# jayleicn/ClipBERT

Measured on AMD Instinct MI355X. Metric: clips/sec/node (2×2 frames, 224px, L_txt=32) at 1/2/4/8 MI355X, higher is better.
Workload: dtype bf16; 1 GPU; MSRVTT retrieval training step (msrvtt_ret_base_resnet50.json; BASELINE configs[1]/[2] family) at the metric's shape: 16 videos x N_clip=2 x N_frame=2 uint8 frames 224px + 2 texts/video (pos+neg, r=2) L_txt=32 per GPU = 32 clips, 64 frames, 64 (text, clip) pairs per step; ImageNorm + fwd + lse-pooling loss + bwd + all-reduce + clip + AdamW in the timed step; clips folded into one forward; mode=train, videos_per_gpu=16, n_clips=2, n_frames=2, img_size=224, txt_len=32, texts_per_video=2, pairs_per_gpu=64, score_agg_func=lse, clips_folded=True, input=uint8 frames in HBM, parallelism=dp1, hip_graph=True, replay_plan=eager hyper-parameter upload + one hipGraph, n_graphs=1, dropout=True

## Files before the change

clipbert_amd/csrc/common.hip:

```cpp
#include "common.h"

#include <stdarg.h>
#include <stdio.h>

namespace {
thread_local char g_err[512] = "";
}

int cb_fail(const char* fmt, ...) {
    va_list ap;
    va_start(ap, fmt);
    vsnprintf(g_err, sizeof(g_err), fmt, ap);
    va_end(ap);
    return -1;
}

int cb_launch_status(const char* what) {
    hipError_t e = hipGetLastError();
    if (e != hipSuccess) return cb_fail("%s: kernel launch failed: %s", what, hipGetErrorString(e));
    return 0;
}

extern "C" const char* cb_last_error(void) { return g_err; }
extern "C" int cb_version(void) { return 18; }
```

clipbert_amd/csrc/gemm.hip:

```cpp

#include "gemm8_impl.h"
#include "gemm_stream_impl.h"
#include <stdio.h>
#include <vector>

using namespace cbgemm;

namespace cbgemm {
extern template int launch_gemm<float, 64, 64, 2>(const GP&, bool, hipStream_t);
extern template int launch_gemm<bf16, 128, 128, 2>(const GP&, bool, hipStream_t);
extern template int launch_gemm<bf16, 128, 64, 2>(const GP&, bool, hipStream_t);
extern template int launch_gemm<bf16, 64, 64, 3>(const GP&, bool, hipStream_t);
extern template int launch_gemm<bf16, 128, 128, 1, 2>(const GP&, bool, hipStream_t);
extern template int launch_gemm_group<float, 64, 64, 2, 1>(const GroupArgs&, int, hipStream_t);
extern template int launch_gemm_group<bf16, 64, 64, 3, 1>(const GroupArgs&, int, hipStream_t);
extern template int launch_gemm_group<bf16, 128, 128, 1, 2>(const GroupArgs&, int, hipStream_t);
#define CB_G8_DECL(BM, BN, WGM, WGN, NST)                                                             \
    extern template int launch_gemm8_fwd<BM, BN, WGM, WGN, NST>(const GP&, int, float*, hipStream_t);   \
    extern template int launch_gemm8_dgrad<BM, BN, WGM, WGN, NST>(const GP&, int, float*, hipStream_t); \
    extern template int launch_gemm8_wgrad<BM, BN, WGM, WGN, NST>(const GP&, int, float*, hipStream_t);
CB_G8_DECL(256, 256, 2, 4, 2)
CB_G8_DECL(128, 256, 2, 4, 3)
CB_G8_DECL(256, 128, 4, 2, 3)
#undef CB_G8_DECL
// ... 208 lines not shown
    const int taps = p.R * p.S;
    const bool tapped = d->a_mode == CB_ROWK_GATHER || d->b_mode == CB_KROW_TAPS || d->b_mode == CB_KROW_GATHER;
    if (tapped) {
        CB_REQUIRE(p.Ct > 0, "cb_gemm: Cin (channels per tap) must be set for conv modes");
        CB_REQUIRE(p.Ct % eps == 0, "cb_gemm: channels per tap (%d) must be a multiple of %d", p.Ct, eps);
    }
    const int64_t lim = 0x7fffffffll;
    bool fast = d->a_bytes > 0 && d->b_bytes > 0 && d->a_bytes < lim && d->b_bytes < lim && aligned16(d->A) && aligned16(d->B);
    if (d->a_mode == CB_ROWK_GATHER) {
        CB_REQUIRE(d->a_tab, "cb_gemm: a_tab missing");
        CB_REQUIRE(d->K == taps * p.Ct, "cb_gemm: K (%d) != R*S*Cin (%d)", d->K, taps * p.Ct);
        fast = fast && (p.R == 1 || d->sH % eps == 0) && (p.S == 1 || d->sW % eps == 0);
    } else if (d->a_mode == CB_ROWK) {
        fast = fast && (d->lda % eps == 0) && (d->K % eps == 0);
    } else {
        const int64_t need = ((int64_t)(d->K - 1) * d->lda + (d->M + eps - 1) / eps * eps) * esz;
        fast = fast && (d->lda % eps == 0) && (d->M % eps == 0 || need <= d->a_bytes);
    }
    if (d->b_mode == CB_ROWK) {
        fast = fast && (d->ldb % eps == 0) && (d->K % eps == 0);
    } else if (d->b_mode == CB_KROW) {
        const int64_t need = ((int64_t)(d->K - 1) * d->ldb + (d->N + eps - 1) / eps * eps) * esz;
        fast = fast && (d->ldb % eps == 0) && (d->N % eps == 0 || need <= d->b_bytes);
    } else if (d->b_mode == CB_KROW_TAPS) {
        CB_REQUIRE(d->K == taps * p.Ct, "cb_gemm: K (%d) != R*S*Ct (%d)", d->K, taps * p.Ct);
        fast = fast && (d->ldb % eps == 0) && (d->N % eps == 0);
    } else {
        CB_REQUIRE(d->b_tab, "cb_gemm: b_tab missing");
        CB_REQUIRE(d->N == taps * p.Ct, "cb_gemm: N (%d) != R*S*Cin (%d)", d->N, taps * p.Ct);
        fast = fast && (p.R == 1 || d->sH % eps == 0) && (p.S == 1 || d->sW % eps == 0);
    }
    p.a_bytes = (uint32_t)(fast ? d->a_bytes : 0);
    p.b_bytes = (uint32_t)(fast ? d->b_bytes : 0);
    CB_REQUIRE(d->tile >= 0 && d->tile <= 9, "cb_gemm: bad tile %d", d->tile);
    CB_REQUIRE(d->xcd_order >= 0 && d->xcd_order <= 2, "cb_gemm: bad xcd_order %d", d->xcd_order);
    CB_REQUIRE(d->dropout_p >= 0.f && d->dropout_p < 1.f, "cb_gemm: dropout_p out of range");
    const int cesz = d->c_f32 ? 4 : esz;
    bool cv = (d->ldc % 4 == 0) && ((reinterpret_cast<uintptr_t>(d->C) % (4 * cesz)) == 0);
    if (d->C2) cv = cv && (d->ldc2 % 4 == 0) && ((reinterpret_cast<uintptr_t>(d->C2) % (4 * esz)) == 0);
    if (d->residual) cv = cv && (d->ldr % 4 == 0) && ((reinterpret_cast<uintptr_t>(d->residual) % (4 * esz)) == 0);
    if (d->mask) cv = cv && (d->ldm % 4 == 0) && ((reinterpret_cast<uintptr_t>(d->mask) % (4 * esz)) == 0);
    if (d->gelu_grad_pre) cv = cv && (d->ld_gelu % 4 == 0) && ((reinterpret_cast<uintptr_t>(d->gelu_grad_pre) % (4 * esz)) == 0);
    if (d->scale) cv = cv && aligned16(d->scale);
    if (d->shift) cv = cv && aligned16(d->shift);
    p.c_vec = cv;
    bool cv8 = cv && (d->N % 8 == 0) && (d->ldc % 8 == 0) && aligned16(d->C);
    if (d->C2) cv8 = cv8 && (d->ldc2 % 8 == 0) && aligned16(d->C2);
    if (d->residual) cv8 = cv8 && (d->ldr % 8 == 0) && aligned16(d->residual);
    if (d->mask) cv8 = cv8 && (d->ldm % 8 == 0) && aligned16(d->mask);
    if (d->gelu_grad_pre) cv8 = cv8 && (d->ld_gelu % 8 == 0) && aligned16(d->gelu_grad_pre);
    out.fast = fast; out.cv8 = cv8;
    out.form = operand_form(d->a_mode, d->b_mode, taps); out.taps = taps;
    out.epi_scale_only = !d->C2 && !d->residual && !d->mask && !d->gelu_grad_pre && d->act == CB_ACT_NONE && !d->relu_after && !d->shift && d->dropout_p <= 0.f;
    out.atomics_ok = out.epi_scale_only && d->c_f32 && d->accumulate == 1;
    return 0;
}

int gemm_validate(const cb_gemm_desc* d, Prepared& pr, bool& empty) {
    empty = false;
    CB_REQUIRE(d != nullptr, "cb_gemm: null descriptor");
    CB_REQUIRE(d->M >= 0 && d->N >= 0 && d->K >= 0, "cb_gemm: negative dims");
    empty = d->M == 0 || d->N == 0;
    return empty ? 0 : gemm_prepare(d, pr);
}

void trace_plan(const cb_gemm_desc* d, const Prepared& pr, const LaunchPlan& lp) {
    if (lp.tile == 9)
        fprintf(stderr, "cb_gemm: M=%d N=%d K=%d modes=%d/%d tile=9 (asked %d) few rows\n", d->M, d->N, d->K, d->a_mode, d->b_mode, d->tile);
    else if (lp.tile == 8)
        fprintf(stderr, "cb_gemm: M=%d N=%d K=%d modes=%d/%d tile=8 (asked %d) stream variant %d\n", d->M, d->N, d->K, d->a_mode, d->b_mode, d->tile, lp.sched);
    else
        fprintf(stderr, "cb_gemm: M=%d N=%d K=%d modes=%d/%d tile=%d (asked %d) form8=%d split=%d ws=%d\n", d->M, d->N, d->K, d->a_mode, d->b_mode,
                lp.picked, d->tile, lp.form8, lp.tile >= 5 ? lp.split_k : pr.p.split_k, (int)lp.slab);
}

int gemm_launch(const cb_gemm_desc* d, const Prepared& pr, const LaunchPlan& lp, hipStream_t st) {
    GP p = pr.p;
    if (lp.tile == 9) return launch_gemm_skinny(d, p, st);
    p.split_k = lp.split_k;
    p.c_vec8 = lp.c_vec8;
    p.xcd_remap = lp.xcd_remap;
    if (lp.tile == 8) return launch_gemm_stream(p, lp.sched, st);
    if (lp.tile >= 5) {
        float* ws = lp.slab ? reinterpret_cast<float*>(d->splitk_ws) : nullptr;
        CB_STAMP_ASSIGN(p, d, lp.tile, p.split_k, lp.sched, 0, 1);
        int rc;
        if (lp.tile == 5) rc = launch8<256, 256, 2, 4, 2>(lp.form8, p, lp.sched - 1, ws, st);
        else if (lp.tile == 6) rc = launch8<128, 256, 2, 4, 3>(lp.form8, p, lp.sched - 1, ws, st);
        else rc = launch8<256, 128, 4, 2, 3>(lp.form8, p, lp.sched - 1, ws, st);
        if (rc != 0 || !ws) return rc;
        GP q = p;
        q.split_k = 1;
        const int64_t chunks = (int64_t)d->M * (d->N / 8);
        hipLaunchKernelGGL(splitk_reduce_kernel, dim3((unsigned)((chunks + 255) / 256), (unsigned)p.batch), dim3(256), 0, st, q, ws, p.split_k);
        return cb_launch_status("cb_gemm (split-K reduce)");
    }
    if (d->dtype == CB_F32) return launch_gemm<float, 64, 64, 2>(p, pr.fast, st);
    CB_STAMP_ASSIGN(p, d, lp.tile, p.split_k, 0, 0, 1);
    if (lp.tile == 4) return launch_gemm<bf16, 128, 128, 1, 2>(p, pr.fast, st);
    if (lp.tile == 1) return launch_gemm<bf16, 128, 128, 2>(p, pr.fast, st);
    if (lp.tile == 3) return launch_gemm<bf16, 128, 64, 2>(p, pr.fast, st);
    return launch_gemm<bf16, 64, 64, 3>(p, pr.fast, st);
}

int gemm_run(const cb_gemm_desc* d, const Prepared& pr, void* stream) {
    LaunchPlan lp;
    const int rc = gemm_choose(d, pr, true, false, lp);
    if (lp.tile != 0 && switches().trace) trace_plan(d, pr, lp);
    return rc != 0 ? rc : gemm_launch(d, pr, lp, cb_stream(stream));
}
}

extern "C" int cb_gemm(const cb_gemm_desc* d, void* stream) {
    Prepared pr;
    bool empty;
// ... 241 lines not shown
```

clipbert_amd/csrc/gemm_choose.h:

```cpp
#pragma once
#include "gemm_impl.h"
#include <cmath>
#include "gemm_tuned.h"
#include "gemm_model.h"

namespace cbgemm {
bool skinny_covers(const cb_gemm_desc* d, const GP& p);
}
using namespace cbgemm;

namespace {
inline int env_int(const char* name, int dflt) { const char* v = getenv(name); return v != nullptr ? atoi(v) : dflt; }
struct Switches {
    bool trace = getenv("CB_GEMM_TRACE") != nullptr;
    bool no_tuned = getenv("CB_GEMM_NO_TUNED") != nullptr;
    bool no_model = getenv("CB_GEMM_NO_MODEL") != nullptr;
    bool no_xcd_remap = getenv("CB_GEMM_NO_XCD_REMAP") != nullptr;
    bool no_stream = getenv("CB_GEMM_NO_STREAM") != nullptr;
    bool no_group = getenv("CB_GEMM_NO_GROUP") != nullptr;
    bool no_skinny = getenv("CB_GEMM_NO_SKINNY") != nullptr;
    bool group_slab_off = env_int("CB_GROUP_SLAB", 1) == 0;
    bool fast_epi_off = env_int("CB_GEMM_FAST_EPI", 1) == 0;
    int wt = env_int("CB_GEMM_WT", 1);
};
// ... 71 lines not shown
    for (int ti = 0; ti < 4; ++ti) {
        if (N <= 64 && ti >= 2) continue;
        consider(ti, split_caller, 0);
        if (free_split)
            for (int s : SPLITS4)
                if (s != split_caller && s <= (p.ktiles / 4 > 1 ? p.ktiles / 4 : 1)) consider(ti, s, 0);
    }
    if (can8)
        for (int ti = 4; ti < 7; ++ti) {
            const int64_t tiles = ((M + MODEL_BM[ti] - 1) / MODEL_BM[ti]) * ((N + MODEL_BN[ti] - 1) / MODEL_BN[ti]) * batch;
            int cand[3] = {1, 0, 0};
            int n = 1;
            for (int target : {256, 512}) {
                const int s = (int)std::lround((double)target / (double)tiles);
                if (s > 1 && p.ktiles / s >= 2 && (int64_t)s * batch * M * N * 4 <= ws_bytes && s != cand[1]) cand[n++] = s;
            }
            for (int i = 0; i < n; ++i) { consider(ti, cand[i], 1); consider(ti, cand[i], 3); }
        }
    return best;
}

int stream_variant(const cb_gemm_desc* d, const Prepared& pr) {
    const GP& p = pr.p;
    if (!pr.fast || !pr.cv8 || d->dtype != CB_BF16 || pr.form != FORM_FWD || p.batch > 1 || p.split_k > 1) return -1;
    if (d->c_f32 || d->accumulate || d->c_rowmap || d->zero_fill_pitch || d->a_rowsum || d->gelu_grad_pre || d->dropout_p > 0.f || d->mask || d->relu_bwd ||
        d->C2 || d->res_rowmap) return -1;
    if (d->K % 8 != 0 || d->M < 64) return -1;
    if ((int64_t)d->M * (d->N > d->K ? d->N : d->K) * 2 >= 0x7fffffffll) return -1;
    if (p.ktiles == 1 && d->N % 256 == 0) return 0;
    if (p.ktiles == 2 && d->N % 128 == 0) return 1;
    return -1;
}

struct LaunchPlan {
    int tile = 0;
    int split_k = 1;
    int sched = 0;
    bool xcd_remap = false;
    bool slab = false;
    bool c_vec8 = false;
    int form8 = 0;
    int picked = 0;
};
struct Pick { int tile = 0, split = 0, sched = 0; };
constexpr int64_t WS_UNLIMITED = (int64_t)1 << 60;
constexpr int STREAM_MIN_ROWS = 32768;

int gemm_choose(const cb_gemm_desc* d, const Prepared& pr, bool use_table, bool assume_ws, LaunchPlan& lp) {
    const Switches& sw = switches();
    const GP& p = pr.p;
    const bool bf = d->dtype == CB_BF16, explicit_tile = d->tile != 0;
    const int split_caller = p.split_k;
    lp = LaunchPlan{};
    const bool covers9 = skinny_covers(d, p);
    CB_REQUIRE(d->tile != 9 || covers9, "cb_gemm: tile 9 (few rows) does not cover this problem (bf16, A k-contiguous, B k-contiguous or aligned reduction-major, no batch / K split / row sums)");
    if (d->tile == 9 || (!explicit_tile && use_table && !sw.no_skinny && covers9 && d->M <= 64)) { lp.tile = 9; return 0; }
    const int sv = stream_variant(d, pr);
    CB_REQUIRE(d->tile != 8 || sv >= 0, "cb_gemm: tile 8 (streaming) does not cover this problem (M=%d N=%d K=%d modes %d/%d)", d->M, d->N, d->K, d->a_mode, d->b_mode);
    const cbgemm::TunedEntry* tabled =
        (bf && use_table && !sw.no_tuned && !d->dgrad_s2) ? cbgemm::tuned_lookup(d->a_mode, d->b_mode, d->M, d->N, d->K, p.batch, pr.taps, split_caller) : nullptr;
    if (!tabled && bf && use_table && !sw.no_tuned && pr.form == FORM_FWD)
        tabled = cbgemm::tuned_lookup(CB_ROWK_GATHER, d->b_mode, d->M, d->N, d->K, p.batch, 1, split_caller);
    if (d->tile == 8 || (!explicit_tile && use_table && !sw.no_stream && !tabled && sv >= 0 && d->M >= STREAM_MIN_ROWS && d->N <= 512)) {
        lp.tile = 8; lp.sched = sv; lp.c_vec8 = true;
        return 0;
    }

    const int form8 = (bf && pr.fast && pr.cv8 && (pr.form != FORM_DGRAD_TAPS || p.Ct % 64 == 0) && !d->res_rowmap && !d->dgrad_s2) ? FORM8_OF[pr.form] : 0;
    const int64_t ws_room = assume_ws ? splitk_payload_bytes(WS_UNLIMITED)
                                      : (d->splitk_ws && aligned16(d->splitk_ws) ? splitk_payload_bytes(d->splitk_ws_bytes) : 0);
    const bool free_split = !explicit_tile && a_reduction_major(pr.form) && pr.atomics_ok;
    const int xcd = d->xcd_order != 0 ? d->xcd_order : (tabled ? tabled->xcd : 0);
    auto model = [&](bool allow8) {
        Pick k;
        if (!bf || sw.no_model) return k;
        const ModelPick mp = model_pick(d, pr, allow8 && form8 != 0, ws_room, free_split && !d->a_rowsum && p.batch == 1);
        k.tile = mp.tile; k.split = (mp.tile >= 5 || mp.split != split_caller) ? mp.split : 0; k.sched = mp.sched;
        return k;
    };
    auto split8 = [&](const Pick& k) { return explicit_tile ? split_caller : (k.split > 0 ? k.split : 1); };
    Pick pick;
    if (explicit_tile) pick.tile = d->tile;
    else if (tabled) pick = Pick{tabled->tile, tabled->new_split, tabled->sched};
    if (pick.tile >= 5 && form8 == 0) pick = Pick{};
    if (pick.tile == 0) pick = model(true);
    if (pick.tile >= 5 && d->sq_slots && split8(pick) > 1) pick = model(false);
    if (pick.tile >= 5) {
        int split = split8(pick);
        if (split > p.ktiles) split = p.ktiles;
// ... 42 lines not shown
```

clipbert_amd/csrc/gemm_impl.h:

```cpp
#pragma once
#include "common.h"
#include <stdlib.h>
#include <type_traits>

namespace cbgemm {


constexpr int NTHREADS = 256;

template <typename T> struct Tr;
template <> struct Tr<bf16> { static constexpr int EPS = 8, BK = 64, SEGS = 8, ROWB = 128, RB = 8; };
template <> struct Tr<float> { static constexpr int EPS = 4, BK = 32, SEGS = 8, ROWB = 144, RB = 4; };

template <typename T> __device__ __forceinline__ int lds_off(int row, int seg);
template <> __device__ __forceinline__ int lds_off<bf16>(int row, int seg) { return row * 128 + ((seg ^ (row & 7)) << 4); }
template <> __device__ __forceinline__ int lds_off<float>(int row, int seg) { return row * 144 + (seg << 4); }

struct GP {
    const void* A; const void* B; void* C; void* C2; const void* residual; const void* mask;
    const void* dact_pre; float* a_rowsum; int64_t ldd;
    int relu_bwd;
    int cls_rows;
    const float* post_scale; const float* post_scale2;
    int batch;
// ... 640 lines not shown

__device__ __forceinline__ void apply_batch(GP& p, TileId& t) {
    if (p.batch <= 1) return;
    const int b = __builtin_amdgcn_readfirstlane(t.bz / p.split_k);
    t.bz -= b * p.split_k;
    const int64_t oa = b * p.bs_a, ob = b * p.bs_b;
    p.A = reinterpret_cast<const unsigned char*>(p.A) + oa;
    p.B = reinterpret_cast<const unsigned char*>(p.B) + ob;
    p.C = reinterpret_cast<unsigned char*>(p.C) + b * p.bs_c;
    if (p.a_bytes) p.a_bytes -= (uint32_t)oa;
    if (p.b_bytes) p.b_bytes -= (uint32_t)ob;
    if (p.a_rowsum) p.a_rowsum += b * p.bs_r;
}

template <int BM, int BK>
__device__ __forceinline__ void dgrad_s2_class(GP& p, TileId& bid) {
    if (p.cls_rows <= 0) return;
    const int cls = 3 - (bid.by & 3);
    bid.by >>= 2;
    const int py = cls >> 1, px = cls & 1;
    p.M = p.cls_rows;
    p.R = 1 + py; p.S = 1 + px;
    p.K = p.R * p.S * p.Ct;
    p.ktiles = (p.K + BK - 1) / BK;
    p.flip = TAP_S2 + 3 * (1 + py) + (1 + px);
    p.c_rowmap += (int64_t)cls * p.cls_rows;
}
inline int dgrad_s2_grid_y(const GP& p, int BM) { return p.cls_rows > 0 ? 4 * ((p.cls_rows + BM - 1) / BM) : (p.M + BM - 1) / BM; }

}
#include "gemm_epilogue.h"
namespace cbgemm {

template <typename T, int BM, int BN, typename LA, typename LB, int PF, bool RS, int OCC>
__device__ __forceinline__ void gemm_tile(GP& p, TileId bid, float* slab = nullptr, int* cnt = nullptr) {
    using X = Tr<T>;
    constexpr int BK = X::BK;
    constexpr int WM = BM / 2, WN = BN / 2, FM = WM / 16, FN = WN / 16;
    constexpr int TILE_A = BM * X::ROWB, TILE_B = BN * X::ROWB;
    constexpr int SMEM_BYTES = 2 * (TILE_A + TILE_B);
    __shared__ __attribute__((aligned(16))) unsigned char smem[SMEM_BYTES];

    const int tid = threadIdx.x, lane = tid & 63, wave = tid >> 6;
    const int wm = wave >> 1, wn = wave & 1;
    CB_STAMP_DECL();
    CB_STAMP(0);
#ifdef CB_STAMPS
    const unsigned stamp_lin = (unsigned)bid.bx + (unsigned)((p.N + BN - 1) / BN) * ((unsigned)bid.by + (unsigned)((p.M + BM - 1) / BM) * (unsigned)bid.bz);
#endif
    const int tile_lin = ((p.batch > 1 ? bid.bz / p.split_k : 0) * ((p.M + BM - 1) / BM) + bid.by) * ((p.N + BN - 1) / BN) + bid.bx;
    apply_batch(p, bid);
    if constexpr (!LA::KROW && LB::KROW) dgrad_s2_class<BM, BK>(p, bid);
    const int m0 = bid.by * BM, n0 = bid.bx * BN;
    const int kt_per = (p.ktiles + p.split_k - 1) / p.split_k;
    const int kt0 = bid.bz * kt_per;
    const int nt = ((kt0 + kt_per < p.ktiles) ? kt0 + kt_per : p.ktiles) - kt0;
    if (nt <= 0) return;

    LA la;
    LB lb;
    {
        Opnd oa = {p.A, p.a_tab, p.lda, p.a_mode, p.a_bytes};
        Opnd ob = {p.B, p.b_tab, p.ldb, p.b_mode, p.b_bytes};
        la.init(p, oa, m0, p.M, kt0, tid);
        lb.init(p, ob, n0, p.N, kt0, tid);
    }
    typename LA::Stage sa[PF];
    typename LB::Stage sb[PF];

    auto load_tiles = [&](typename LA::Stage& xa, typename LB::Stage& xb) {
        la.template load<false>(xa, p);
        lb.template load<false>(xb, p);
    };
    auto load_tiles_checked = [&](typename LA::Stage& xa, typename LB::Stage& xb) {
        la.template load<true>(xa, p);
        lb.template load<true>(xb, p);
    };
    auto store_tiles = [&](const typename LA::Stage& xa, const typename LB::Stage& xb, int buf) {
        unsigned char* As = smem + buf * (TILE_A + TILE_B);
        la.store(xa, As, tid);
        lb.store(xb, As + TILE_A, tid);
    };

    f32x4 acc[FM][FN];
#pragma unroll
    for (int i = 0; i < FM; ++i)
#pragma unroll
        for (int j = 0; j < FN; ++j) { f32x4 z = {0.f, 0.f, 0.f, 0.f}; acc[i][j] = z; }
    f32x4 accr[RS ? FM : 1];
#pragma unroll
    for (int i = 0; i < (RS ? FM : 1); ++i) { f32x4 z = {0.f, 0.f, 0.f, 0.f}; accr[i] = z; }
    const bool rs_on = RS && p.a_rowsum != nullptr && bid.bx == 0 && wn == 0;

#pragma unroll
    for (int s = 0; s < PF; ++s)
        if (s < nt) load_tiles_checked(sa[s], sb[s]);
    constexpr bool DGRAD = sizeof(T) == 2 && !LA::KROW && LB::KROW;
    constexpr int EPF = !DGRAD ? 0 : (BM * BN <= 128 * 64 ? 2 : (OCC >= 2 ? 1 : 0));
    EpiPre<BM, BN, EPF != 1> epre;
    const bool epf_on = EPF != 0 && p.c_vec8 && (EPF == 2 ? p.relu_bwd != 0 : (p.dact_pre != nullptr && !p.relu_bwd));
    if constexpr (EPF != 0) {
        if (epf_on) epi_prefetch<T, BM, BN, EPF != 1>(p, epre, m0, n0, tid);
    }
    store_tiles(sa[0], sb[0], 0);
    if (PF < nt) load_tiles_checked(sa[0], sb[0]);
    __syncthreads();
    CB_STAMP(1);

    auto compute_tile = [&](int buf) {
        const unsigned char* As = smem + buf * (TILE_A + TILE_B);
        const unsigned char* Bs = As + TILE_A;
        if constexpr (sizeof(T) == 2) {
#pragma unroll
            for (int kk = 0; kk < BK / 32; ++kk) {
                bf16x8 af[FM], bfr[FN];
#pragma unroll
                for (int i = 0; i < FM; ++i) {
                    if constexpr (LA::TR) af[i] = tr_frag<BM>(As, wm * WM + i * 16, kk, lane);
                    else af[i] = *reinterpret_cast<const bf16x8*>(As + lds_off<T>(wm * WM + i * 16 + (lane & 15), kk * 4 + (lane >> 4)));
                }
#pragma unroll
                for (int j = 0; j < FN; ++j) {
                    if constexpr (LB::TR) bfr[j] = tr_frag<BN>(Bs, wn * WN + j * 16, kk, lane);
                    else bfr[j] = *reinterpret_cast<const bf16x8*>(Bs + lds_off<T>(wn * WN + j * 16 + (lane & 15), kk * 4 + (lane >> 4)));
                }
#pragma unroll
                for (int i = 0; i < FM; ++i)
#pragma unroll
                    for (int j = 0; j < FN; ++j)
                        acc[i][j] = __builtin_amdgcn_mfma_f32_16x16x32_bf16(bfr[j], af[i], acc[i][j], 0, 0, 0);
                if constexpr (RS) {
// ... 39 lines not shown
            compute_tile(t & 1);
            store_tiles(sa[S1], sb[S1], (t + 1) & 1);
            load_tiles(sa[S1], sb[S1]);
            __syncthreads();
            ++t;
        }
    }
    while (t < nt) {
#pragma unroll
        for (int s = 0; s < PF; ++s) {
            if (t < nt) {
                const int S1 = (s + 1) % PF;
                compute_tile(t & 1);
                if (t + 1 < nt) {
                    store_tiles(sa[S1], sb[S1], (t + 1) & 1);
                    if (t + 1 + PF < nt) load_tiles_checked(sa[S1], sb[S1]);
                }
                __syncthreads();
                ++t;
            }
        }
    }

    if constexpr (RS) {
        if (rs_on && (lane >> 4) == 0) {
#pragma unroll
            for (int i = 0; i < FM; ++i) {
                const int m = m0 + wm * WM + i * 16 + lane;
                if (m < p.M) atomicAdd(p.a_rowsum + m, accr[i][0]);
            }
        }
    }
    CB_STAMP(2);
    if (slab != nullptr && p.split_k > 1) {
        __shared__ int s_last;
        constexpr int SC1 = 16;
        const int tile_lin = bid.by * ((p.N + BN - 1) / BN) + bid.bx;
        const int parts = (p.ktiles + kt_per - 1) / kt_per;
        float* const base = slab + ((int64_t)p.slab_base + (int64_t)tile_lin * p.split_k) * (BM * BN);
        {
            const rsrc_t rs = __builtin_amdgcn_make_buffer_rsrc(base + (int64_t)bid.bz * (BM * BN), (short)0, BM * BN * 4, 0x00020000);
#pragma unroll
            for (int i = 0; i < BM / 32; ++i)
#pragma unroll
                for (int j = 0; j < BN / 32; ++j) {
                    union { f32x4 f; u32x4 r; } u;
                    u.f = acc[i][j];
                    __builtin_amdgcn_raw_buffer_store_b128(u.r, rs, (uint32_t)(((i * (BN / 32) + j) * NTHREADS + tid) * 16), 0, SC1);
                }
        }
        __builtin_amdgcn_s_waitcnt(0x0f70);
        __syncthreads();
        if (tid == 0) s_last = atomicAdd(cnt + p.cnt_base + tile_lin, 1) == parts - 1;
        __syncthreads();
        if (!s_last) {
            CB_STAMP(3);
            CB_STAMP_FLUSH(p, stamp_lin, tid);
            return;
        }
#pragma unroll
        for (int i = 0; i < BM / 32; ++i)
#pragma unroll
            for (int j = 0; j < BN / 32; ++j) { f32x4 z = {0.f, 0.f, 0.f, 0.f}; acc[i][j] = z; }
#pragma unroll 2
        for (int z = 0; z < parts; ++z) {
            const rsrc_t rs = __builtin_amdgcn_make_buffer_rsrc(base + (int64_t)z * (BM * BN), (short)0, BM * BN * 4, 0x00020000);
#pragma unroll
            for (int i = 0; i < BM / 32; ++i)
#pragma unroll
                for (int j = 0; j < BN / 32; ++j) {
                    union { u32x4 r; f32x4 f; } u;
                    u.r = __builtin_amdgcn_raw_buffer_load_b128(rs, (uint32_t)(((i * (BN / 32) + j) * NTHREADS + tid) * 16), 0, SC1);
                    acc[i][j] += u.f;
                }
        }
        if (tid == 0) atomicExch(cnt + p.cnt_base + tile_lin, 0);
        p.split_k = 1;
    }
    constexpr int FORM_ = LA::KROW ? 0 : (LB::KROW ? 2 : 1);
    if constexpr (EPF != 0) tile_epilogue<T, BM, BN, SMEM_BYTES, EPF, false, FORM_>(p, acc, smem, m0, n0, tid, epre, epf_on);
    else tile_epilogue<T, BM, BN, SMEM_BYTES, 0, LA::KROW, FORM_>(p, acc, smem, m0, n0, tid, EpiPre<BM, BN, true>{}, false, tile_lin);
    CB_STAMP(3);
    CB_STAMP_FLUSH(p, stamp_lin, tid);
}

template <typename T, int BM, int BN, typename LA, typename LB, int PF, bool RS = false, int OCC = 1>
__global__ void __launch_bounds__(256, OCC) gemm_kernel(GP p) {
    gemm_tile<T, BM, BN, LA, LB, PF, RS, OCC>(p, tile_id(p));
}

#ifdef CB_STAMPS
constexpr int GROUP_MAX = 9;
#else
constexpr int GROUP_MAX = 10;
#endif
struct GroupArgs {
    int n, xcd_remap;
    int tile_end[GROUP_MAX];
    float* slab;
    int* cnt;
    GP g[GROUP_MAX];
};
static_assert(sizeof(GroupArgs) + 256 <= 4096, "kernel arguments (+ the hidden ones) are limited to 4 KiB");

template <int BM, int BN>
__device__ __forceinline__ int group_locate(const GroupArgs& ga, TileId& bid) {
    const unsigned total = gridDim.x;
    unsigned lin = blockIdx.x;
    if (ga.xcd_remap) {
        const unsigned xcd = lin & 7u, i = lin >> 3;
        const unsigned q = total >> 3, r = total & 7u;
        lin = (xcd < r ? xcd * (q + 1) : r * (q + 1) + (xcd - r) * q) + i;
    }
    int pi = 0;
    while (pi + 1 < ga.n && lin >= (unsigned)ga.tile_end[pi]) ++pi;
    const unsigned local = lin - (pi > 0 ? (unsigned)ga.tile_end[pi - 1] : 0u);
    const unsigned gx = (unsigned)((ga.g[pi].N + BN - 1) / BN), gy = (unsigned)((ga.g[pi].M + BM - 1) / BM);
    bid.bx = (int)(local % gx);
    const unsigned rest = local / gx;
    bid.by = (int)(rest % gy);
    bid.bz = (int)(rest / gy);
// ... 51 lines not shown
            }
        }
    }
    template <bool CHECK> __device__ __forceinline__ void issue(const GP& p, unsigned char* tile, int wave) {
        if constexpr (GATHER) {
            const bool kv = rr < p.R;
            const uint32_t koff = (uint32_t)(rr * (int)p.sH + ss * (int)p.sW + c) * 2u;
#pragma unroll
            for (int i = 0; i < NI; ++i) {
                const bool v = kv && (unsigned)(ih[i] + rr) < (unsigned)p.H && (unsigned)(iw[i] + ss) < (unsigned)p.W;
                dma16(rs, tile + (i * 4 + wave) * 1024, v ? voff[i] + koff : OOB);
            }
            if (p.Ct >= X::BK) {
                c += X::BK;
                if (c >= p.Ct) { c -= p.Ct; if (++ss == p.S) { ss = 0; ++rr; } }
            } else {
                ss += X::BK / p.Ct;
                while (ss >= p.S) { ss -= p.S; ++rr; }
            }
        } else {
#pragma unroll
            for (int i = 0; i < NI; ++i) {
                uint32_t o32 = voff[i];
                if (CHECK && krem <= 0) o32 = OOB;
                dma16(rs, tile + (i * 4 + wave) * 1024, o32);
                voff[i] += X::BK * 2u;
            }
            krem -= X::BK;
        }
    }
};

inline bool aligned16(const void* p) { return (reinterpret_cast<uintptr_t>(p) & 15) == 0; }

template <typename T, int BM, int BN, int PF, int OCC, typename LA, typename LB, bool RS = false>
int launch_k(const GP& p, hipStream_t st) {
    dim3 grid((p.N + BN - 1) / BN, dgrad_s2_grid_y(p, BM), p.split_k * (p.batch > 1 ? p.batch : 1));
    hipLaunchKernelGGL((gemm_kernel<T, BM, BN, LA, LB, PF, RS, OCC>), grid, dim3(NTHREADS), 0, st, p);
    return cb_launch_status("cb_gemm");
}
template <typename T, int BM, int BN, int PF, int OCC, typename LA, typename LB>
int launch_wgrad(const GP& p, hipStream_t st) {
    if (p.a_rowsum) return launch_k<T, BM, BN, PF, OCC, LA, LB, true>(p, st);
    return launch_k<T, BM, BN, PF, OCC, LA, LB, false>(p, st);
}

template <typename T, int BM, int BN, int PF, int OCC = 1>
int launch_gemm(const GP& p, bool fast, hipStream_t st) {
    const bool a_krow = p.a_mode == CB_KROW;
    const bool b_krow = p.b_mode != CB_ROWK;
    if (a_krow && !b_krow) return cb_fail("cb_gemm: unsupported operand mode combination (A KROW with B ROWK)");
    if (fast) {
        const int taps = p.R * p.S;
        if constexpr (sizeof(T) == 2) {
            if constexpr (BN < 128) {
                if (p.a_mode == CB_ROWK && (p.b_mode == CB_KROW || (p.b_mode == CB_KROW_TAPS && taps == 1)))
                    return launch_k<T, BM, BN, PF, OCC, RowkFast<T, BM, false>, KrowTr<BN, KM_PLAIN>>(p, st);
                if (p.a_mode == CB_ROWK_GATHER && p.b_mode == CB_KROW_TAPS && p.Ct % Tr<bf16>::BK == 0)
                    return launch_k<T, BM, BN, PF, OCC, RowkFast<T, BM, true>, KrowTr<BN, KM_TAPS>>(p, st);
            }
            if (p.a_mode == CB_KROW && p.b_mode == CB_KROW)
                return launch_wgrad<T, BM, BN, PF, OCC, KrowTr<BM, KM_PLAIN>, KrowTr<BN, KM_PLAIN>>(p, st);
            if (p.a_mode == CB_KROW && p.b_mode == CB_KROW_GATHER)
                return launch_k<T, BM, BN, PF, OCC, KrowTr<BM, KM_PLAIN>, KrowTr<BN, KM_GATHER>>(p, st);
        }
        if (p.a_mode == CB_ROWK && p.b_mode == CB_ROWK)
// ... 60 lines not shown
```

clipbert_amd/modeling/encoder.py:

```python
from collections import namedtuple
from types import SimpleNamespace
from typing import Optional

import numpy as np
import torch
from torch import nn

from .. import ops
from ..ops import ACT_GELU, ACT_TANH, KROW
from .modules import BertEmbeddings, BertEncoder, BertPooler, VisualInputEmbedding, _cfg_get, as_config
from .runtime import _SITE_ATTN, _SITE_EMB, _SITE_OUT, _SITE_PIXEL, _SITE_POOL, _SITE_SELF_OUT, Runtime, _pick_split, _seed


class ClipBertBaseModel(nn.Module):
    def __init__(self, config):
        super().__init__()
        config = as_config(config)
        assert _cfg_get(config, "hidden_act", "gelu") == "gelu", "only the exact-erf GELU of base_model.json is implemented"
        assert config.hidden_size // config.num_attention_heads == 64, "attention kernels are built for head size 64"
        self.config = config
        self.embeddings = BertEmbeddings(config)
        self.visual_embeddings = VisualInputEmbedding(config)
        self.encoder = BertEncoder(config)
        self.pooler = BertPooler(config)
        self.rt: Optional[Runtime] = None

    def get_input_embeddings(self):
        return self.embeddings.word_embeddings

    def forward(self, text_input_ids, visual_inputs, attention_mask, src_row=None, pooled_dropout=False, text_repeat=1):
        seq, pooled = _EncoderFn.apply(self.rt.anchor, visual_inputs, self, text_input_ids, attention_mask, src_row,
                                       pooled_dropout, text_repeat)
        b = text_input_ids.shape[0] * text_repeat
        return seq.view(b, -1, self.config.hidden_size), pooled


_LayerSaved = namedtuple("_LayerSaved", "qkv ctx lse a_pre mean1 rstd1 hsave o_pre mean2 rstd2")


def _drop_p(model, training, key="hidden_dropout_prob"):
    return float(_cfg_get(model.config, key, 0.0)) if training else 0.0


def encoder_forward(model: ClipBertBaseModel, grid, ids, mask, src_row, pooled_dropout, save, text_repeat=1):
# ... 38 lines not shown
    pre = torch.empty(M, d, dtype=dt, device=dev) if save else None
    mean0, rstd0 = torch.empty(2, M, dtype=torch.float32, device=dev) if save else (None, None)
    emb, vemb = model.embeddings, model.visual_embeddings
    ids_c = ids.contiguous()
    ops.text_embed_fwd(ids_c, bank.compute(emb.word_embeddings.weight), bank.compute(emb.position_embeddings.weight),
                       bank.compute(emb.token_type_embeddings.weight)[0], emb.LayerNorm.weight, emb.LayerNorm.bias, x, pre,
                       mean0, rstd0, lt, L, eps, attn_mask=mask_c, key_mask=key_mask, repeat=text_repeat)
    grid_c = grid.contiguous()
    ops.visual_embed_fwd(grid_c, src_row, sel, bank.compute(vemb.row_position_embeddings.weight),
                         bank.compute(vemb.col_position_embeddings.weight), bank.compute(vemb.token_type_embeddings.weight)[0],
                         vemb.LayerNorm.weight, vemb.LayerNorm.bias, x, pre, mean0, rstd0, bsz, lv, lt, L, eps, key_mask=key_mask)
    if p_h > 0:
        ops.dropout(x, p_h, _seed(_SITE_EMB, 0, fwd_i), rt.seed_dev, out=x)
    layers = []
    for li, layer in enumerate(model.encoder.layer):
        att, so, it, ou = layer.attention.self, layer.attention.output, layer.intermediate, layer.output
        wqkv = bank.compute_span(att.query.weight, att.value.weight, (3 * d, d))
        bqkv = bank.master_span(att.query.bias, att.value.bias, (3 * d,))
        qkv = torch.empty(M, 3 * d, dtype=dt, device=dev)
        ops.gemm(x, wqkv, M, 3 * d, d, out=qkv, shift=bqkv)
        ctx, lse = ops.attention_fwd(qkv, key_mask, bsz, L, nh, save_lse=save, dropout_p=p_a,
                                     dropout_seed=_seed(_SITE_ATTN, li, fwd_i), seed_ptr=rt.seed_dev, out=stk.ctx[li] if save else None)
        a_pre = torch.empty(M, d, dtype=dt, device=dev)
        ops.gemm(ctx, bank.compute(so.dense.weight), M, d, d, out=a_pre, shift=so.dense.bias, residual=x, dropout_p=p_h,
                 dropout_seed=_seed(_SITE_SELF_OUT, li, fwd_i), seed_ptr=rt.seed_dev)
        a, mean1, rstd1 = ops.layernorm_fwd(a_pre, so.LayerNorm.weight, so.LayerNorm.bias, eps, save_stats=save,
                                            out=stk.a[li] if save else None)
        hact = stk.hact[li] if save else torch.empty(M, ff, dtype=dt, device=dev)
        hsave = torch.empty(M, ff, dtype=dt, device=dev) if save else None
        ops.gemm(a, bank.compute(it.dense.weight), M, ff, d, out=hact, shift=it.dense.bias,
                 act=ops.ACT_GELU_SAVE_GRAD if save else ACT_GELU, out2=hsave)
        o_pre = torch.empty(M, d, dtype=dt, device=dev)
        ops.gemm(hact, bank.compute(ou.dense.weight), M, d, ff, out=o_pre, shift=ou.dense.bias, residual=a, dropout_p=p_h,
                 dropout_seed=_seed(_SITE_OUT, li, fwd_i), seed_ptr=rt.seed_dev)
        out, mean2, rstd2 = ops.layernorm_fwd(o_pre, ou.LayerNorm.weight, ou.LayerNorm.bias, eps, save_stats=save,
                                              out=stk.x[li + 1] if (save and li + 1 < nl) else None)
        if save:
            layers.append(_LayerSaved(qkv, ctx, lse, a_pre, mean1, rstd1, hsave, o_pre, mean2, rstd2))
        x = out
    pooled = torch.empty(bsz, d, dtype=dt, device=dev)
    p_pool = p_h if pooled_dropout else 0.0
    pooled_raw = torch.empty(bsz, d, dtype=dt, device=dev) if (save and p_pool > 0) else None
    pw = model.pooler.dense
    drop = dict(dropout_p=p_pool, dropout_seed=_seed(_SITE_POOL, 0, fwd_i), seed_ptr=rt.seed_dev) if pooled_raw is None else {}
    ops.gemm(x, bank.compute(pw.weight), bsz, d, d, out=pooled if pooled_raw is None else pooled_raw, lda=L * d, shift=pw.bias, act=ACT_TANH, **drop)
    if pooled_raw is not None:
        ops.dropout(pooled_raw, p_pool, _seed(_SITE_POOL, 0, fwd_i), rt.seed_dev, out=pooled)
    pack = None
    if save:
        pack = SimpleNamespace(layers=layers, x_final=x, pooled=pooled, pooled_raw=pooled_raw, p_pool=p_pool, pre=pre,
                               mean0=mean0, rstd0=rstd0, ids=ids_c, key_mask=key_mask, src_row=src_row, sel=sel, bsz=bsz,
                               lt=lt, lv=lv, L=L, grid_shape=tuple(grid.shape), p_h=p_h, p_a=p_a, stk=stk, fwd_i=fwd_i, text_repeat=text_repeat)
    return x, pooled, pack


def _linear_wgrad(g, x, m, n, k, gw, gb, ldx=None, gather=None, defer_bias=False):
    rides = gw is not None and gather is None
    if gw is not None:
        split, tile = _pick_split(n, k, m)
        xkw = gather if gather is not None else dict(b_mode=KROW, ldb=ldx if ldx is not None else x.stride(0), a_rowsum=gb)
        ops.gemm(g, x, n, k, m, out=gw, a_mode=KROW, lda=g.stride(0), **xkw, accumulate=True, split_k=split, tile=tile)
    owed = None if rides else gb
    if owed is not None and not defer_bias:
        ops.colsum(g, owed, m, n)
        owed = None
    return owed

# ... 96 lines not shown
        if pk.pooled_raw is not None:
            g = ops.dropout(g, pk.p_pool, _seed(_SITE_POOL, 0, pk.fwd_i), rt.seed_dev)
            g = ops.act_bwd(ACT_TANH, g, pk.pooled_raw)
        else:
            g = ops.act_bwd(ACT_TANH, g, pk.pooled)
        pw = model.pooler.dense
        _linear_wgrad(g, pk.x_final, bsz, d, d, bank.grad_image(pw.weight), bank.grad_image(pw.bias), ldx=L * d)
        ops.gemm(g, bank.compute(pw.weight), bsz, d, d, out=dx, b_mode=KROW, ldc=L * d, accumulate=True)
    nl, stk = len(pk.layers), pk.stk
    ln_off = _ln_offsets(model, dev)
    nb = ops.ln_part_blocks(M)
    ln_part = torch.empty(2 * nl, nb, 2, d, dtype=torch.float32, device=dev) if ln_off is not None else None

    def ln_bwd(slot, dy, xpre, ln, mean, rstd, seed, g_out):
        keep = dict(dx2=g_out) if pk.p_h > 0 else dict(dx=g_out)
        if ln_part is not None:
            d_pre, d_drop = ops.layernorm_bwd_part(dy, xpre, ln.weight, mean, rstd, ln_part[slot], pk.p_h, seed, rt.seed_dev, **keep)
        else:
            d_pre, d_drop = ops.layernorm_bwd(dy, xpre, ln.weight, mean, rstd, bank.grad_image(ln.weight), bank.grad_image(ln.bias), pk.p_h,
                                              seed, rt.seed_dev, **keep)
        return d_pre, d_drop if d_drop is not None else d_pre

    gs = SimpleNamespace(out=torch.empty(nl, M, d, dtype=dt, device=dev), hp=torch.empty(nl, M, ff, dtype=dt, device=dev),
                         att=torch.empty(nl, M, d, dtype=dt, device=dev), qkv=torch.empty(nl, M, 3 * d, dtype=dt, device=dev))
    for li in range(nl - 1, -1, -1):
        layer = model.encoder.layer[li]
        att, so, it, ou = layer.attention.self, layer.attention.output, layer.intermediate, layer.output
        sv = pk.layers[li]
        d_o_pre, g = ln_bwd(2 * li + 1, dx, sv.o_pre, ou.LayerNorm, sv.mean2, sv.rstd2, _seed(_SITE_OUT, li, pk.fwd_i), gs.out[li])
        dhp = gs.hp[li]
        ops.gemm(g, bank.compute(ou.dense.weight), M, ff, d, out=dhp, b_mode=KROW, gelu_grad_pre=sv.hsave,
                 act=ops.ACT_SAVED_GRAD)
        da = torch.empty(M, d, dtype=dt, device=dev)
        ops.gemm(dhp, bank.compute(it.dense.weight), M, d, ff, out=da, b_mode=KROW, residual=d_o_pre)
        d_a_pre, g = ln_bwd(2 * li, da, sv.a_pre, so.LayerNorm, sv.mean1, sv.rstd1, _seed(_SITE_SELF_OUT, li, pk.fwd_i), gs.att[li])
        dctx = torch.empty(M, d, dtype=dt, device=dev)
        ops.gemm(g, bank.compute(so.dense.weight), M, d, d, out=dctx, b_mode=KROW)
        dqkv = ops.attention_bwd(sv.qkv, pk.key_mask, sv.ctx, dctx, sv.lse, bsz, L, nh, pk.p_a, _seed(_SITE_ATTN, li, pk.fwd_i), rt.seed_dev,
                                 out=gs.qkv[li])
        wqkv = bank.compute_span(att.query.weight, att.value.weight, (3 * d, d))
        dx = torch.empty(M, d, dtype=dt, device=dev)
        ops.gemm(dqkv, wqkv, M, d, 3 * d, out=dx, b_mode=KROW, residual=d_a_pre)
    if ln_part is not None:
        ops.ln_partials_reduce(ln_part, bank.grad, ln_off[0], ln_off[1])
    _encoder_wgrads(model, pk, gs, M)
    if pk.p_h > 0:
        dx = ops.dropout(dx, pk.p_h, _seed(_SITE_EMB, 0, pk.fwd_i), rt.seed_dev)
    emb, vemb = model.embeddings, model.visual_embeddings
    dpre = torch.empty(M, d, dtype=dt, device=dev)
    ops.layernorm_bwd(dx, pk.pre, emb.LayerNorm.weight, pk.mean0, pk.rstd0, bank.grad_image(emb.LayerNorm.weight),
                      bank.grad_image(emb.LayerNorm.bias), dx=dpre, rows=bsz * lt, seg=(lt, L, 0))
    ops.layernorm_bwd(dx, pk.pre, vemb.LayerNorm.weight, pk.mean0, pk.rstd0, bank.grad_image(vemb.LayerNorm.weight),
                      bank.grad_image(vemb.LayerNorm.bias), dx=dpre, rows=bsz * lv, seg=(lv, L, lt))
    we = emb.word_embeddings
    ops.text_embed_bwd(dpre, pk.ids, bank.grad_image(we.weight), bank.grad_image(emb.position_embeddings.weight),
                       bank.grad_image(emb.token_type_embeddings.weight)[0], lt, L,
                       we.padding_idx if we.padding_idx is not None else -1, repeat=pk.text_repeat)
    dgrid = ops.zeros(pk.grid_shape, torch.float32, dev)
    ops.visual_embed_bwd(dpre, pk.src_row, pk.sel, dgrid, bank.grad_image(vemb.row_position_embeddings.weight),
                         bank.grad_image(vemb.col_position_embeddings.weight), bank.grad_image(vemb.token_type_embeddings.weight)[0],
                         bsz, lv, lt, L)
    return dgrid if dt == torch.float32 else ops.cast(dgrid, torch.empty(pk.grid_shape, dtype=dt, device=dev))


class _EncoderFn(torch.autograd.Function):
    @staticmethod
    def forward(ctx, anchor, grid, model, ids, mask, src_row, pooled_dropout, text_repeat=1):
        save = ctx.needs_input_grad[0]
        ctx.set_materialize_grads(False)
        seq, pooled, pack = encoder_forward(model, grid, ids, mask, src_row, pooled_dropout, save, text_repeat)
        ctx.model, ctx.pack = model, pack
        if save:
            model.rt.pending_encoder_nodes += 1
        return seq, pooled

# ... 7 lines not shown
```

clipbert_amd/modeling/runtime.py:

```python
from typing import Optional

import torch

from .. import ops
from ..params import ParamBank

_HOOK = {"encoder": "after_encoder_backward", "cnn": "after_res5_backward"}


def even_pixel_rows(n, h, w):
    return (torch.arange(n).view(n, 1, 1) * (h * w) + (torch.arange(0, h, 2)).view(1, -1, 1) * w + torch.arange(0, w, 2).view(1, 1, -1)).reshape(-1)


def parity_class_rows(n, h, w):
    even = even_pixel_rows(n, h, w)
    return torch.cat([even + py * w + px for py in (0, 1) for px in (0, 1)])


def even_pixel_index(n, h, w):
    even = even_pixel_rows(n, h, w)
    t = torch.full((n * h * w,), -1, dtype=torch.int64)
    t[even] = torch.arange(even.numel())
    return t


class Runtime:
    def __init__(self):
        self.bank: Optional[ParamBank] = None
        self.dtype = torch.bfloat16
        self.tables = {}
        self.rowmaps = {}
        self.seed_dev: Optional[torch.Tensor] = None
# ... 24 lines not shown
        key = (n, oh, ow, stride, pad, sN, sH, sW, str(device))
        t = self.tables.get(key)
        if t is None:
            t = ops.build_pixel_table(n, oh, ow, stride, pad, sN, sH, sW, device)
            self.tables[key] = t
        return t

    def strided_rowmap(self, n, h, w, oh, ow, stride, device):
        key = (n, h, w, oh, ow, stride, str(device))
        t = self.rowmaps.get(key)
        if t is None:
            t = (torch.arange(n).view(n, 1, 1) * (h * w) + (torch.arange(oh) * stride).view(1, oh, 1) * w
                 + (torch.arange(ow) * stride).view(1, 1, ow)).reshape(-1).to(torch.int32).to(device)
            self.rowmaps[key] = t
        return t

    def rowmap(self, kind, n, h, w, device):
        key = (kind.__name__, n, h, w, str(device))
        t = self.rowmaps.get(key)
        if t is None:
            t = self.rowmaps[key] = kind(n, h, w).to(torch.int32).to(device)
        return t


def _pick_split(mo, no, kred):
    ktiles = (kred + 63) // 64
    b64 = ((mo + 63) // 64) * ((no + 63) // 64)
    if b64 >= 200 or ktiles < 64:
        return 1, 0
    split = max(1, min(ktiles // 8, (400 + b64 // 2) // b64))
    return split, 0


_SITE_EMB, _SITE_ATTN, _SITE_SELF_OUT, _SITE_OUT, _SITE_POOL, _SITE_REG = 1, 2, 3, 4, 5, 6
_SITE_PIXEL = 7


def _seed(site, layer=0, fwd=0):
    return ((site * 1000003 + layer * 7919) * 2654435761 + fwd * 0x9E3779B97F4A7C15) % (1 << 62)
```

Measured before the change: 4287 clips/s.

## Add intra-workgroup K-split GEMM tile for deep-K encoder GEMMs

Adds a new GEMM variant (tile 10) where a 512-thread workgroup runs two wave groups, each reducing half of the K range for a 128x64 output tile. The partial accumulators are summed through shared memory before one epilogue runs. The encoder's FFN output GEMM and two deep-K data-gradient GEMMs select it when the tile count is small (at most 256 tiles) and K is at least 1536. This targets under-filled GPUs on small-M, large-K GEMMs without needing a split-K workspace and a separate reduce kernel. The cost is doubled LDS per workgroup, an extra barrier and shared-memory reduction, and lower occupancy.

```diff
diff --git a/clipbert_amd/csrc/common.hip b/clipbert_amd/csrc/common.hip
--- a/clipbert_amd/csrc/common.hip
+++ b/clipbert_amd/csrc/common.hip
@@ -22,4 +22,4 @@
 }
 
 extern "C" const char* cb_last_error(void) { return g_err; }
-extern "C" int cb_version(void) { return 18; }
+extern "C" int cb_version(void) { return 19; }
diff --git a/clipbert_amd/csrc/gemm.hip b/clipbert_amd/csrc/gemm.hip
--- a/clipbert_amd/csrc/gemm.hip
+++ b/clipbert_amd/csrc/gemm.hip
@@ -264,7 +264,7 @@
     }
     p.a_bytes = (uint32_t)(fast ? d->a_bytes : 0);
     p.b_bytes = (uint32_t)(fast ? d->b_bytes : 0);
-    CB_REQUIRE(d->tile >= 0 && d->tile <= 9, "cb_gemm: bad tile %d", d->tile);
+    CB_REQUIRE(d->tile >= 0 && d->tile <= 10, "cb_gemm: bad tile %d", d->tile);
     CB_REQUIRE(d->xcd_order >= 0 && d->xcd_order <= 2, "cb_gemm: bad xcd_order %d", d->xcd_order);
     CB_REQUIRE(d->dropout_p >= 0.f && d->dropout_p < 1.f, "cb_gemm: dropout_p out of range");
     const int cesz = d->c_f32 ? 4 : esz;
@@ -301,6 +301,8 @@
         fprintf(stderr, "cb_gemm: M=%d N=%d K=%d modes=%d/%d tile=9 (asked %d) few rows\n", d->M, d->N, d->K, d->a_mode, d->b_mode, d->tile);
     else if (lp.tile == 8)
         fprintf(stderr, "cb_gemm: M=%d N=%d K=%d modes=%d/%d tile=8 (asked %d) stream variant %d\n", d->M, d->N, d->K, d->a_mode, d->b_mode, d->tile, lp.sched);
+    else if (lp.tile == 10)
+        fprintf(stderr, "cb_gemm: M=%d N=%d K=%d modes=%d/%d tile=10 (asked %d) K halves\n", d->M, d->N, d->K, d->a_mode, d->b_mode, d->tile);
     else
         fprintf(stderr, "cb_gemm: M=%d N=%d K=%d modes=%d/%d tile=%d (asked %d) form8=%d split=%d ws=%d\n", d->M, d->N, d->K, d->a_mode, d->b_mode,
                 lp.picked, d->tile, lp.form8, lp.tile >= 5 ? lp.split_k : pr.p.split_k, (int)lp.slab);
@@ -313,6 +315,10 @@
     p.c_vec8 = lp.c_vec8;
     p.xcd_remap = lp.xcd_remap;
     if (lp.tile == 8) return launch_gemm_stream(p, lp.sched, st);
+    if (lp.tile == 10) {
+        CB_STAMP_ASSIGN(p, d, lp.tile, 1, 0, 0, 1);
+        return launch_gemm_khalves(p, st);
+    }
     if (lp.tile >= 5) {
         float* ws = lp.slab ? reinterpret_cast<float*>(d->splitk_ws) : nullptr;
         CB_STAMP_ASSIGN(p, d, lp.tile, p.split_k, lp.sched, 0, 1);
diff --git a/clipbert_amd/csrc/gemm_choose.h b/clipbert_amd/csrc/gemm_choose.h
--- a/clipbert_amd/csrc/gemm_choose.h
+++ b/clipbert_amd/csrc/gemm_choose.h
@@ -127,6 +127,13 @@
     return -1;
 }
 
+bool khalves_covers(const cb_gemm_desc* d, const Prepared& pr) {
+    const GP& p = pr.p;
+    if (d->dtype != CB_BF16 || !pr.fast || (pr.form != FORM_FWD && pr.form != FORM_DGRAD)) return false;
+    if (p.batch > 1 || p.split_k > 1 || d->a_rowsum || d->res_rowmap || d->dgrad_s2 || d->zero_fill_pitch || d->sq_slots) return false;
+    return d->K > 0 && d->K % Tr<bf16>::BK == 0 && p.ktiles % 2 == 0;
+}
+
 struct LaunchPlan {
     int tile = 0;
     int split_k = 1;
@@ -150,6 +157,14 @@
     const bool covers9 = skinny_covers(d, p);
     CB_REQUIRE(d->tile != 9 || covers9, "cb_gemm: tile 9 (few rows) does not cover this problem (bf16, A k-contiguous, B k-contiguous or aligned reduction-major, no batch / K split / row sums)");
     if (d->tile == 9 || (!explicit_tile && use_table && !sw.no_skinny && covers9 && d->M <= 64)) { lp.tile = 9; return 0; }
+    if (d->tile == 10) {
+        CB_REQUIRE(khalves_covers(d, pr), "cb_gemm: tile 10 (K halves in the workgroup) does not cover this problem (bf16 fast path, forward or data-gradient "
+                   "form without gather, an even number of whole 64-deep K tiles, no batch / K split / row sums / row-mapped residual / dgrad_s2 / zero fill; "
+                   "M=%d N=%d K=%d modes %d/%d)", d->M, d->N, d->K, d->a_mode, d->b_mode);
+        lp.tile = lp.picked = 10; lp.c_vec8 = pr.cv8;
+        lp.xcd_remap = !sw.no_xcd_remap && d->xcd_order != 2;
+        return 0;
+    }
     const int sv = stream_variant(d, pr);
     CB_REQUIRE(d->tile != 8 || sv >= 0, "cb_gemm: tile 8 (streaming) does not cover this problem (M=%d N=%d K=%d modes %d/%d)", d->M, d->N, d->K, d->a_mode, d->b_mode);
     const cbgemm::TunedEntry* tabled =
diff --git a/clipbert_amd/csrc/gemm_impl.h b/clipbert_amd/csrc/gemm_impl.h
--- a/clipbert_amd/csrc/gemm_impl.h
+++ b/clipbert_amd/csrc/gemm_impl.h
@@ -696,16 +696,20 @@
 #include "gemm_epilogue.h"
 namespace cbgemm {
 
-template <typename T, int BM, int BN, typename LA, typename LB, int PF, bool RS, int OCC>
+template <typename T, int BM, int BN, typename LA, typename LB, int PF, bool RS, int OCC, int KG = 1>
 __device__ __forceinline__ void gemm_tile(GP& p, TileId bid, float* slab = nullptr, int* cnt = nullptr) {
     using X = Tr<T>;
     constexpr int BK = X::BK;
     constexpr int WM = BM / 2, WN = BN / 2, FM = WM / 16, FN = WN / 16;
     constexpr int TILE_A = BM * X::ROWB, TILE_B = BN * X::ROWB;
     constexpr int SMEM_BYTES = 2 * (TILE_A + TILE_B);
-    __shared__ __attribute__((aligned(16))) unsigned char smem[SMEM_BYTES];
-
-    const int tid = threadIdx.x, lane = tid & 63, wave = tid >> 6;
+    static_assert(KG == 1 || (KG == 2 && sizeof(T) == 2 && BM == 128 && BN == 64 && !RS && !LA::KROW), "two wave groups: bf16 128x64, forward / data gradient");
+    static_assert(KG == 1 || FM * FN * NTHREADS * 16 <= SMEM_BYTES, "group 1's accumulators do not fit its region");
+    __shared__ __attribute__((aligned(16))) unsigned char smem_all[KG * SMEM_BYTES];
+
+    const int grp = KG == 1 ? 0 : __builtin_amdgcn_readfirstlane((int)(threadIdx.x / NTHREADS));
+    unsigned char* const smem = smem_all + grp * SMEM_BYTES;
+    const int tid = KG == 1 ? (int)threadIdx.x : (int)(threadIdx.x % NTHREADS), lane = tid & 63, wave = tid >> 6;
     const int wm = wave >> 1, wn = wave & 1;
     CB_STAMP_DECL();
     CB_STAMP(0);
@@ -716,8 +720,8 @@
     apply_batch(p, bid);
     if constexpr (!LA::KROW && LB::KROW) dgrad_s2_class<BM, BK>(p, bid);
     const int m0 = bid.by * BM, n0 = bid.bx * BN;
-    const int kt_per = (p.ktiles + p.split_k - 1) / p.split_k;
-    const int kt0 = bid.bz * kt_per;
+    const int kt_per = KG == 1 ? (p.ktiles + p.split_k - 1) / p.split_k : p.ktiles / KG;
+    const int kt0 = (KG == 1 ? bid.bz : grp) * kt_per;
     const int nt = ((kt0 + kt_per < p.ktiles) ? kt0 + kt_per : p.ktiles) - kt0;
     if (nt <= 0) return;
 
@@ -760,7 +764,7 @@
     for (int s = 0; s < PF; ++s)
         if (s < nt) load_tiles_checked(sa[s], sb[s]);
     constexpr bool DGRAD = sizeof(T) == 2 && !LA::KROW && LB::KROW;
-    constexpr int EPF = !DGRAD ? 0 : (BM * BN <= 128 * 64 ? 2 : (OCC >= 2 ? 1 : 0));
+    constexpr int EPF = (!DGRAD || KG != 1) ? 0 : (BM * BN <= 128 * 64 ? 2 : (OCC >= 2 ? 1 : 0));
     EpiPre<BM, BN, EPF != 1> epre;
     const bool epf_on = EPF != 0 && p.c_vec8 && (EPF == 2 ? p.relu_bwd != 0 : (p.dact_pre != nullptr && !p.relu_bwd));
     if constexpr (EPF != 0) {
@@ -866,7 +870,7 @@
         }
     }
     CB_STAMP(2);
-    if (slab != nullptr && p.split_k > 1) {
+    if (KG == 1 && slab != nullptr && p.split_k > 1) {
         __shared__ int s_last;
         constexpr int SC1 = 16;
         const int tile_lin = bid.by * ((p.N + BN - 1) / BN) + bid.bx;
@@ -889,7 +893,7 @@
         __syncthreads();
         if (!s_last) {
             CB_STAMP(3);
-            CB_STAMP_FLUSH(p, stamp_lin, tid);
+            CB_STAMP_FLUSH(p, stamp_lin, (int)threadIdx.x);
             return;
         }
 #pragma unroll
@@ -911,16 +915,39 @@
         if (tid == 0) atomicExch(cnt + p.cnt_base + tile_lin, 0);
         p.split_k = 1;
     }
+    if constexpr (KG == 2) {
+        unsigned char* const part = smem_all + SMEM_BYTES;
+        if (grp == 1) {
+#pragma unroll
+            for (int i = 0; i < FM; ++i)
+#pragma unroll
+                for (int j = 0; j < FN; ++j) *reinterpret_cast<f32x4*>(part + ((i * FN + j) * NTHREADS + tid) * 16) = acc[i][j];
+        }
+        __syncthreads();
+        if (grp == 0) {
+#pragma unroll
+            for (int i = 0; i < FM; ++i)
+#pragma unroll
+                for (int j = 0; j < FN; ++j) acc[i][j] = acc[i][j] + *reinterpret_cast<const f32x4*>(part + ((i * FN + j) * NTHREADS + tid) * 16);
+        } else {
+            p.M = 0;
+        }
+    }
     constexpr int FORM_ = LA::KROW ? 0 : (LB::KROW ? 2 : 1);
     if constexpr (EPF != 0) tile_epilogue<T, BM, BN, SMEM_BYTES, EPF, false, FORM_>(p, acc, smem, m0, n0, tid, epre, epf_on);
     else tile_epilogue<T, BM, BN, SMEM_BYTES, 0, LA::KROW, FORM_>(p, acc, smem, m0, n0, tid, EpiPre<BM, BN, true>{}, false, tile_lin);
     CB_STAMP(3);
-    CB_STAMP_FLUSH(p, stamp_lin, tid);
+    CB_STAMP_FLUSH(p, stamp_lin, (int)threadIdx.x);
 }
 
 template <typename T, int BM, int BN, typename LA, typename LB, int PF, bool RS = false, int OCC = 1>
 __global__ void __launch_bounds__(256, OCC) gemm_kernel(GP p) {
     gemm_tile<T, BM, BN, LA, LB, PF, RS, OCC>(p, tile_id(p));
+}
+
+template <typename LA, typename LB, int PF>
+__global__ void __launch_bounds__(2 * NTHREADS, 2) gemm_khalves_kernel(GP p) {
+    gemm_tile<bf16, 128, 64, LA, LB, PF, false, 1, 2>(p, tile_id(p));
 }
 
 #ifdef CB_STAMPS
@@ -1038,6 +1065,8 @@
 };
 
 inline bool aligned16(const void* p) { return (reinterpret_cast<uintptr_t>(p) & 15) == 0; }
+
+int launch_gemm_khalves(const GP& p, hipStream_t st);
 
 template <typename T, int BM, int BN, int PF, int OCC, typename LA, typename LB, bool RS = false>
 int launch_k(const GP& p, hipStream_t st) {
diff --git a/clipbert_amd/csrc/gemm_inst_bf16_128x64_kh.hip b/clipbert_amd/csrc/gemm_inst_bf16_128x64_kh.hip
--- /dev/null
+++ b/clipbert_amd/csrc/gemm_inst_bf16_128x64_kh.hip
@@ -0,0 +1,11 @@
+#include "gemm_impl.h"
+
+namespace cbgemm {
+int launch_gemm_khalves(const GP& p, hipStream_t st) {
+    const dim3 grid((p.N + 63) / 64, (p.M + 127) / 128, 1), block(2 * NTHREADS);
+    using RA = RowkFast<bf16, 128, false>;
+    if (p.b_mode == CB_ROWK) hipLaunchKernelGGL((gemm_khalves_kernel<RA, RowkFast<bf16, 64, false>, 2>), grid, block, 0, st, p);
+    else hipLaunchKernelGGL((gemm_khalves_kernel<RA, KrowTr<64, KM_PLAIN>, 2>), grid, block, 0, st, p);
+    return cb_launch_status("cb_gemm (tile 10)");
+}
+}
diff --git a/clipbert_amd/modeling/encoder.py b/clipbert_amd/modeling/encoder.py
--- a/clipbert_amd/modeling/encoder.py
+++ b/clipbert_amd/modeling/encoder.py
@@ -9,7 +9,7 @@
 from .. import ops
 from ..ops import ACT_GELU, ACT_TANH, KROW
 from .modules import BertEmbeddings, BertEncoder, BertPooler, VisualInputEmbedding, _cfg_get, as_config
-from .runtime import _SITE_ATTN, _SITE_EMB, _SITE_OUT, _SITE_PIXEL, _SITE_POOL, _SITE_SELF_OUT, Runtime, _pick_split, _seed
+from .runtime import _SITE_ATTN, _SITE_EMB, _SITE_OUT, _SITE_PIXEL, _SITE_POOL, _SITE_SELF_OUT, Runtime, _pick_khalves, _pick_split, _seed
 
 
 class ClipBertBaseModel(nn.Module):
@@ -114,7 +114,7 @@
                  act=ops.ACT_GELU_SAVE_GRAD if save else ACT_GELU, out2=hsave)
         o_pre = torch.empty(M, d, dtype=dt, device=dev)
         ops.gemm(hact, bank.compute(ou.dense.weight), M, d, ff, out=o_pre, shift=ou.dense.bias, residual=a, dropout_p=p_h,
-                 dropout_seed=_seed(_SITE_OUT, li, fwd_i), seed_ptr=rt.seed_dev)
+                 dropout_seed=_seed(_SITE_OUT, li, fwd_i), seed_ptr=rt.seed_dev, tile=_pick_khalves(M, d, ff, dt))
         out, mean2, rstd2 = ops.layernorm_fwd(o_pre, ou.LayerNorm.weight, ou.LayerNorm.bias, eps, save_stats=save,
                                               out=stk.x[li + 1] if (save and li + 1 < nl) else None)
         if save:
@@ -277,7 +277,7 @@
         ops.gemm(g, bank.compute(ou.dense.weight), M, ff, d, out=dhp, b_mode=KROW, gelu_grad_pre=sv.hsave,
                  act=ops.ACT_SAVED_GRAD)
         da = torch.empty(M, d, dtype=dt, device=dev)
-        ops.gemm(dhp, bank.compute(it.dense.weight), M, d, ff, out=da, b_mode=KROW, residual=d_o_pre)
+        ops.gemm(dhp, bank.compute(it.dense.weight), M, d, ff, out=da, b_mode=KROW, residual=d_o_pre, tile=_pick_khalves(M, d, ff, dt))
         d_a_pre, g = ln_bwd(2 * li, da, sv.a_pre, so.LayerNorm, sv.mean1, sv.rstd1, _seed(_SITE_SELF_OUT, li, pk.fwd_i), gs.att[li])
         dctx = torch.empty(M, d, dtype=dt, device=dev)
         ops.gemm(g, bank.compute(so.dense.weight), M, d, d, out=dctx, b_mode=KROW)
@@ -285,7 +285,7 @@
                                  out=gs.qkv[li])
         wqkv = bank.compute_span(att.query.weight, att.value.weight, (3 * d, d))
         dx = torch.empty(M, d, dtype=dt, device=dev)
-        ops.gemm(dqkv, wqkv, M, d, 3 * d, out=dx, b_mode=KROW, residual=d_a_pre)
+        ops.gemm(dqkv, wqkv, M, d, 3 * d, out=dx, b_mode=KROW, residual=d_a_pre, tile=_pick_khalves(M, d, 3 * d, dt))
     if ln_part is not None:
         ops.ln_partials_reduce(ln_part, bank.grad, ln_off[0], ln_off[1])
     _encoder_wgrads(model, pk, gs, M)
diff --git a/clipbert_amd/modeling/runtime.py b/clipbert_amd/modeling/runtime.py
--- a/clipbert_amd/modeling/runtime.py
+++ b/clipbert_amd/modeling/runtime.py
@@ -1,3 +1,4 @@
+import os
 from typing import Optional
 
 import torch
@@ -88,6 +89,18 @@
     return split, 0
 
 
+_KHALVES_OFF = os.environ.get("CB_GEMM_NO_KHALVES") is not None
+
+
+def _pick_khalves(m, n, k, dtype=torch.bfloat16):
+    if _KHALVES_OFF or dtype != torch.bfloat16 or n <= 0 or n % 64 != 0 or k % 64 != 0:
+        return 0
+    ktiles = k // 64
+    if ktiles % 2 != 0 or k < 1536:
+        return 0
+    return 10 if ((m + 127) // 128) * (n // 64) <= 256 else 0
+
+
 _SITE_EMB, _SITE_ATTN, _SITE_SELF_OUT, _SITE_OUT, _SITE_POOL, _SITE_REG = 1, 2, 3, 4, 5, 6
 _SITE_PIXEL = 7
 
```

Result: no change. 4320 clips/s, median of 4 (+0.8%).
